# prakharg24/yoloret

Hardware: AMD Instinct MI355X
Metric: images/sec (+ p50 per-image ms) MobileNetV2-0.75x @416, 1/2/4/8 MI355X (higher is better)
Workload: dtype f32; 1 GPU; mobilenetv2x75 @416, batch 64 per GPU, fp32, random weights (SURVEY 8(d) recipe; parity tests run the variance-preserving recipe, see DESIGN.md 5), C=20: forward + decode + per-class NMS + pack; 3 steps in flight (each step = one whole batch on its own HIP stream and workspace); global_batch=64, parallelism=dp1 (image-sharded)

## Files before the change

### yoloret_amd/compiler.py

```python
import ctypes
import os

import numpy as np

from . import runtime as rt


def round_up(v, m):
    return (v + m - 1) // m * m


NO_ARENA_REUSE = os.environ.get('YOLORET_NO_ARENA_REUSE', '0') != '0'


class Buf:
    def __init__(self, bid, h, w, c, ld, external_slot=-1, name='', dtype=0):
        self.id, self.h, self.w, self.c, self.ld = bid, h, w, c, ld
        self.external_slot = external_slot
        self.name = name
        self.dtype = dtype
        self.elems = h * w * ld
        self.bytes = self.elems * rt.ESIZE[dtype]
        self.first_def = None
        self.last_use = -1
# ... 858 lines not shown
                out.append(m16)
                i += 2
            else:
                out.append(c)
                i += 1
            continue
        ok = (d is not None and c.kind == rt.OP_POINTWISE and c.dtype == 0 and c.act in ('relu6', 'none', 'swish', 'leaky') and 'scale' in c.params
              and c.res is None and not getattr(c, 'stride', 0) and not (c.se_reduced & rt.PWF_F32_MFMA) and not getattr(c, 'accounted_in', None)
              and all(s_.xform in ('identity', 'up2', 'maxpool2', 'maxpool4', 'up2_add') for s_ in c.srcs)
              and (c.gate is None or (len(c.srcs) == 1 and c.srcs[0].xform == 'identity'))
              and kp >= 16 and c.cout % 4 == 0 and c.out.external_slot < 0 and c.out.id not in output_buf_ids and readers.get(id(c.out), 0) == 1
              and d.kind == rt.OP_DEPTHWISE and d.dtype == 0 and d.k == 3 and d.stride == 1 and len(d.srcs) == 1 and d.srcs[0].buf is c.out
              and d.srcs[0].xform == 'identity' and d.srcs[0].c == c.cout and d.act in ('swish', 'relu6', 'none') and d.out.ld % 4 == 0
              and d.out.dtype == 0 and not (c.h == 1 and c.w == 1) and (d.gate is not None or FUSE_HEAD_ALL)
              and block_name(c.name) + '_head' not in nosplit)
        if not ok:
            if c.kind == rt.OP_POINTWISE and block_name(c.name) + '_head' in nosplit:
                c.se_reduced |= rt.PWF_F32_MFMA
            out.append(c)
            i += 1
            continue
        F, ldf = c.cout, round_up(c.cout, 4)
        m = OpRec(rt.OP_HEAD, block_name(c.name) + '_head', act=d.act, h=d.h, w=d.w, cin=c.cin, cout=F, k=3 | rt.ACT[c.act] << rt.HEAD_ACT_SHIFT, stride=1,
                  srcs=list(c.srcs), out=d.out, res=c.gate, macs=c.macs + d.macs, dtype=0)
        m.fused = [c, d]
        if getattr(c, 'folded_projection', None):
            m.folded_projection = c.folded_projection
        m.params = {'wgt': c.params['wgt'], 'scale': c.params['scale'], 'shift': c.params['shift']}
        dp = d.params
        kseg = [s_.c for s_ in c.srcs if s_.xform != 'up2_add']
        nk = sum((c_ + 31) // 32 for c_ in kseg)
        nt = 2 if nk <= 4 else 1
        bname_h = block_name(c.name)
        ksrc = [s_ for s_ in c.srcs if s_.xform != 'up2_add']
        hs_shape = HEAD_STREAM_ONLY or (20 <= d.h <= 30 and d.w <= 28 and nk >= 5) or (d.h < 20 and d.w <= 14 and 5 <= nk <= 8)
        stream = (HEAD_STREAM and stream_ok and hs_shape and not SE_TAIL and (not HEAD_STREAM_ONLY or bname_h in HEAD_STREAM_ONLY)
                  and all(s_.xform in ('identity', 'maxpool2', 'up2_add') for s_ in c.srcs)
                  and all(s_.xform != 'up2_add' for s_ in c.srcs[:-1]) and 1 <= len(ksrc) <= 3 and F % 32 == 0 and c.act in ('relu6', 'none')
                  and nk <= (7 if head_stream_geometry(d.h, d.w)[0] == 2 else 11) and not (c.gate is not None and (len(ksrc) != 1 or ksrc[0].xform != 'identity'))
                  and all(s_.buf.ld % 4 == 0 for s_ in ksrc)
                  and 4 * nk * 2048 + 2 * 10 * (2 if d.h >= 20 else 1) * 2048 + F * 11 * 4 + F * 4 <= 160 * 1024)
        walk = (not stream and HEAD_WALK and all(s_.xform in ('identity', 'up2_add') for s_ in c.srcs) and len(kseg) <= 3 and nk <= HEAD_WALK_MAX_NK and F % 16 == 0 and (F // 16 // nt) % 4 == 0
                and F // 16 % nt == 0 and c.act in ('relu6', 'none') and not (c.gate is not None and len(kseg) != len(c.srcs)) and F * 11 * 4 <= 64 * 1024)
        if walk or stream:
            m.k |= rt.HEAD_STREAM if stream else rt.HEAD_WALK
            cp = c.params

            def planes(wd, cp=cp, kseg=kseg, F=F):
                return head_pack((cp['wgt'][1](wd)[:F] * cp['scale'][1](wd)[:F, None]).astype(np.float32), kseg)

            def tab(wd, cp=cp, dp=dp, F=F):
                T = F // 16
                o = np.zeros((T, 11, 16), np.float32)
                o[:, :9] = (dp['wgt'][1](wd).reshape(9, -1)[:, :F] * dp['scale'][1](wd)[None, :F]).astype(np.float32).reshape(9, T, 16).transpose(1, 0, 2)
                o[:, 9], o[:, 10] = dp['shift'][1](wd)[:F].reshape(T, 16), cp['shift'][1](wd)[:F].reshape(T, 16)
                return o
            m.params = {'wgt': (((F // 16) * nk * 512,), planes), 'scale': c.params['scale'], 'wgt2': ((F // 16, 11, 16), tab)}
        elif all(s_.xform in ('identity', 'up2', 'up2_add') for s_ in c.srcs) and len(kseg) <= 3 and HEAD_DMA:
            m.k |= rt.HEAD_PLANES
            m.params['wgt'] = ((((F + 15) // 16) * nk * 512,), lambda wd, wf=c.params['wgt'][1], kseg=kseg: head_pack(wf(wd), kseg))

        def dw_rows(wd, dp=dp, F=F, ldf=ldf):
            o = np.zeros((10, ldf), np.float32)
            o[:9, :F] = (dp['wgt'][1](wd).reshape(9, -1)[:, :F] * dp['scale'][1](wd)[None, :F]).astype(np.float32)
            o[9, :F] = dp['shift'][1](wd)[:F]
            return o
        if not (walk or stream):
            m.params['wgt2'] = ((10, ldf), dw_rows)
        if d.gate is not None:
            nsy, nsx = (head_stream_rows(d.h, d.w), 1) if stream else (head_walk_rows(d.h, d.w), 1) if walk else head_regions(d.h, d.w)
            part = d.gate
            part.h, part.w = nsy * nsx, 1
            part.elems = part.h * part.w * part.ld
            part.bytes = part.elems * rt.ESIZE[part.dtype]
            m.gate, m.se_reduced = part, nsy * nsx
        if hasattr(c, 'accounting_srcs'):
            m.fused[0].accounting_srcs = c.accounting_srcs
        out.append(m)
        i += 2
    return out


def se_tail_into_producers(ops):
    producer_of_sums = {id(op.gate): op for op in ops
                        if op.gate is not None and (op.kind == rt.OP_HEAD or (op.kind == rt.OP_DEPTHWISE and not dw_uses_lds_form(op)))}
    drop = set()
    for fc in ops:
        if fc.kind != rt.OP_SE_FC or len(fc.srcs) != 1 or not fc.k > 0:
            continue
        P = producer_of_sums.get(id(fc.srcs[0].buf))
        if P is None or P.gate_out is not None or fc.out.external_slot >= 0:
            continue
        if P.kind == rt.OP_HEAD and (P.k & rt.HEAD_STREAM) == rt.HEAD_STREAM:
            continue
        C, R = fc.cin, fc.se_reduced
        ldc = round_up(C, 4)
        if C != P.cout or fc.k != P.h * P.w or ldc + R > SE_TAIL_LDS:
            continue
        fp = fc.params

        def se_w(wd, fp=fp, R=R, ldc=ldc):
            return np.concatenate([np.asarray(fp['wgt'][1](wd), np.float32).ravel(), np.asarray(fp['wgt2'][1](wd), np.float32).ravel(),
                                   np.asarray(fp['b1'][1](wd), np.float32).ravel(), np.asarray(fp['b2'][1](wd), np.float32).ravel()])
        P.params['se_w'] = ((ldc * round_up(R, 4) + R * ldc + round_up(R, 4) + ldc,), se_w)
        P.gate_out, P.se_hidden = fc.out, R
        P.macs += fc.macs
        P.absorbed = list(getattr(P, 'absorbed', ())) + [fc]
        drop.add(id(fc))
    return [op for op in ops if id(op) not in drop]



def mbr_pack(we_t, e_scale, e_shift, dw, d_scale, d_shift, wp_t, p_scale, p_shift):
    cexp = dw.shape[1] // 16 * 16
    if wp_t is None:
        wp_t, p_scale, p_shift = np.zeros((0, cexp), np.float32), np.zeros(0, np.float32), np.zeros(0, np.float32)
    cout = wp_t.shape[0]
    cin = we_t.shape[1] // 8 * 8
    assert dw.shape[1] >= cexp and cexp % 16 == 0 and cin % 16 in (0, 8), (dw.shape, we_t.shape)
    T, TO, KE, nmain = cexp // 16, (cout + 15) // 16, cin // 4, cin // 16
    wef = (we_t[:cexp, :cin] * e_scale[:cexp, None]).astype(np.float32)
    wpf = np.zeros((16 * TO, cexp), np.float32)
    wpf[:cout] = (wp_t[:, :cexp] * p_scale[:cout, None]).astype(np.float32)
    lane = np.arange(64)
    m, g = lane % 16, lane // 16
    wa = np.zeros((T, KE + 4 * TO, 64), np.float32)
    for j in range(T):
        for q in range(KE):
            c, s = divmod(q, 4)
            kidx = 16 * c + 4 * g + s if c < nmain else 16 * nmain + 2 * g + s
            wa[j, q] = wef[16 * j + m, kidx]
        for t in range(TO):
            for s in range(4):
                wa[j, KE + 4 * t + s] = wpf[16 * t + m, 16 * j + 4 * g + s]
    tab = np.zeros((T, 11, 16), np.float32)
    tab[:, :9] = (dw[:, :cexp] * d_scale[None, :cexp]).astype(np.float32).reshape(9, T, 16).transpose(1, 0, 2)
    tab[:, 9], tab[:, 10] = d_shift[:cexp].reshape(T, 16), e_shift[:cexp].reshape(T, 16)
    b2 = np.zeros(16 * TO, np.float32)
    b2[:cout] = p_shift[:cout]
    return wa, tab, b2


def mbs_wave_pairs(T, nw):
    ntl, r = divmod(T, nw)
    pairs, t0 = [], 0
    for w in range(nw):
        nt = ntl + (1 if w < r else 0)
        for q in range(0, nt, 2):
            pairs.append((t0 + q, t0 + q + 1 if q + 1 < nt else None))
        t0 += nt
    return pairs


def mbs_pack(we_t, e_scale, e_shift, dw, d_scale, d_shift, wp_t, p_scale, p_shift, nw):
    _, tab, b2 = mbr_pack(we_t, e_scale, e_shift, dw, d_scale, d_shift, wp_t, p_scale, p_shift)
    cexp = dw.shape[1] // 16 * 16
    if wp_t is None:
        wp_t, p_scale, nw = np.zeros((0, cexp), np.float32), np.zeros(0, np.float32), 0
    cout, cin = wp_t.shape[0], we_t.shape[1] // 8 * 8
    T, TO, NKE = cexp // 16, (cout + 15) // 16, (cin + 31) // 32
    wef = np.zeros((cexp, 32 * NKE), np.float32)
    wef[:, :cin] = (we_t[:cexp, :cin] * e_scale[:cexp, None]).astype(np.float32)
    wpf = np.zeros((16 * TO, cexp), np.float32)
    wpf[:cout] = (wp_t[:, :cexp] * p_scale[:cout, None]).astype(np.float32)
    assert max(np.abs(wef).max(), np.abs(wpf).max() if wpf.size else 0.0) < 60000.0, 'mbs_pack: a weight beyond the float16 range'

    def planes(x):
        h = x.astype(np.float16)
        m = ((x - h.astype(np.float32)) * np.float32(2048.0)).astype(np.float16)
        return h, m
    lane = np.arange(64)
    m_, g = lane % 16, lane // 16
    i8 = np.arange(8)
    ex = np.zeros((T, NKE, 2, 64, 8), np.float16)
    for j in range(T):
        for c in range(NKE):
            v = wef[(16 * j + m_)[:, None], 32 * c + 8 * g[:, None] + i8[None, :]]
            ex[j, c, 0], ex[j, c, 1] = planes(v)
    pairs = mbs_wave_pairs(T, nw) if nw else []
    pr = np.zeros((len(pairs), TO, 2, 64, 8), np.float16)
    for q, (ta, tb) in enumerate(pairs):
        for t in range(TO):
            v = np.zeros((64, 8), np.float32)
            v[:, :4] = wpf[(16 * t + m_)[:, None], 16 * ta + 4 * g[:, None] + i8[None, :4]]
            if tb is not None:
                v[:, 4:] = wpf[(16 * t + m_)[:, None], 16 * tb + 4 * g[:, None] + i8[None, :4]]
            pr[q, t, 0], pr[q, t, 1] = planes(v)
    wa = np.concatenate([ex.ravel(), pr.ravel()]).view(np.float32)
    return wa, tab, b2


def mbk_chunk_words(cin, cout):
    return (4 * ((cin + 31) // 32) + 2 * ((cout + 15) // 16)) * 256 + 512


def mbk_pack(we_t, e_scale, e_shift, dw, d_scale, d_shift, wp_t, p_scale, p_shift):
    wa, tab, b2 = mbs_pack(we_t, e_scale, e_shift, dw, d_scale, d_shift, wp_t, p_scale, p_shift, 1)
    cexp = dw.shape[1] // 16 * 16
    cout, cin = wp_t.shape[0], we_t.shape[1] // 8 * 8
    T, TO, NKE = cexp // 16, (cout + 15) // 16, (cin + 31) // 32
    NQ = (T + 1) // 2
    ex = wa[:T * NKE * 512].reshape(T, NKE * 512)
    pr = wa[T * NKE * 512:].reshape(NQ, TO * 512)
    cw = mbk_chunk_words(cin, cout)
    out = np.zeros((NQ, cw), np.float32)
    for q in range(NQ):
        o = 0
        for t in (2 * q, 2 * q + 1):
            if t < T:
                out[q, o:o + NKE * 512] = ex[t]
            o += NKE * 512
        out[q, o:o + TO * 512] = pr[q]
        o += TO * 512
        for t in (2 * q, 2 * q + 1):
            if t < T:
                out[q, o:o + 176] = tab[t].ravel()
            o += 176
    return out.ravel(), b2


def mbk_segs(stride, h, pad_t, nw, rows):
    ho = (h + stride - 1) // stride
    if stride == 1:
        nr = nw * rows
        return 1 if h <= nr else (h - nr + nr - 3) // (nr - 2) + 1
    s = 0
    while True:
        ylast = s * (nw - 1) + nw - 1
        end = ylast if 2 * ylast - pad_t + 2 >= h else ylast - 1
        if end >= ho - 1:
            return s + 1
        s += 1


def pad_to(fn, n, ld):
    def f(wd):
        o = np.zeros(ld, np.float32)
        o[:n] = fn(wd)[:n]
        return o
    return f


def bn_pair(prm, n, ld):
    return lambda wd: np.concatenate([pad_to(prm['scale'][1], n, ld)(wd), pad_to(prm['shift'][1], n, ld)(wd)])


def block_arrays(wd, ep, dp, pp=None):
    proj = (pp['wgt'][1](wd), pp['scale'][1](wd), pp['shift'][1](wd)) if pp is not None else (None, None, None)
    return (ep['wgt'][1](wd), ep['scale'][1](wd), ep['shift'][1](wd), dp['wgt'][1](wd).reshape(9, -1), dp['scale'][1](wd), dp['shift'][1](wd)) + proj


def packed(pack, which, ep, dp, pp=None, *extra):
    return lambda wd: pack(*block_arrays(wd, ep, dp, pp), *extra)[which]


def stem_pair_rows(prm, taps, c1p):
    def f(wd):
        sc = pad_to(prm['scale'][1], c1p, c1p)(wd)
        w = (prm['wgt'][1](wd).reshape(taps, -1)[:, :c1p] * sc[None]).astype(np.float32)
        rows = np.concatenate([w, np.ones((1, c1p), np.float32), pad_to(prm['shift'][1], c1p, c1p)(wd)[None]])
        return np.ascontiguousarray(rows.reshape(taps + 2, c1p // 2, 2).transpose(1, 0, 2)).reshape(c1p // 2, -1)
    return ((c1p // 2, (taps + 2) * 2), f)


def stemblock_params(e, d, p):
    c1p, cout, cop = round_up(e.cout, 4), p.cout, round_up(p.cout, 8)

    def proj_w(wd, pw=p.params['wgt'][1]):
        o = np.zeros((c1p, cop), np.float32)
        o[:, :cout] = pw(wd)[:, :c1p].T
        return o
    return {'wgt': stem_pair_rows(e.params, 27, c1p), 'wgt2': stem_pair_rows(d.params, 9, c1p), 'b1': ((c1p, cop), proj_w),
            'b2': ((2 * cop,), bn_pair(p.params, cout, cop))}


def stemblock_mfma_params(e, d, p, dtype):
    c1, cout = e.cout, p.cout
    c1m, com = round_up(c1, 32), round_up(cout, 16)
    korder = [g * 9 + i_ for g in range(3) for i_ in range(8)] + [i_ * 9 + 8 for i_ in range(3)]

    def stem_w(wd, ew=e.params['wgt'][1]):
        o = np.zeros((c1m, 32), np.float32)
        o[:c1, :27] = ew(wd)[korder, :c1].T
        return o

    def dw_rows(wd, dp=d.params):
        o = np.zeros((10, c1m), np.float32)
        sc = dp['scale'][1](wd)[:c1]
        o[:9, :c1] = (dp['wgt'][1](wd).reshape(9, -1)[:, :c1] * sc[None]).astype(np.float32)
        o[9, :c1] = dp['shift'][1](wd)[:c1]
        return o

    def proj_m(wd, pw=p.params['wgt'][1]):
        o = np.zeros((com, c1m), np.float32)
        o[:cout, :c1] = pw(wd)[:cout, :c1]
        return o
    return {'wgt': ((c1m, 32), stem_w, dtype), 'scale': ((c1m,), pad_to(e.params['scale'][1], c1, c1m)),
            'shift': ((c1m,), pad_to(e.params['shift'][1], c1, c1m)), 'wgt2': ((10, c1m), dw_rows), 'b1': ((com, c1m), proj_m, dtype),
            'b2': ((2 * com,), bn_pair(p.params, cout, com))}


def mbh_params(ep, dp, pp, cin, cexp, cout, k, dtype):
    kk, cexp_p, kp, ldo = k * k, round_up(cexp, 32), round_up(cin, 32), round_up(cout, 8)

    def expand_wt(wd):
        o = np.zeros((cexp_p, kp), np.float32)
        o[:cexp, :cin] = ep['wgt'][1](wd)[:, :cin]
        return o

    def chunk_params(wd):
        o = np.zeros((kk + 4, cexp_p), np.float32)
        o[:kk, :cexp] = dp['wgt'][1](wd)[:, :cexp]
        o[kk, :cexp], o[kk + 1, :cexp] = dp['scale'][1](wd)[:cexp], dp['shift'][1](wd)[:cexp]
        o[kk + 2, :cexp], o[kk + 3, :cexp] = ep['scale'][1](wd)[:cexp], ep['shift'][1](wd)[:cexp]
        return o

    def project_wt(wd):
        o = np.zeros((cout, cexp_p), np.float32)
        o[:, :cexp] = pp['wgt'][1](wd)[:, :cexp]
        return o

    def project_bn(wd):
        o = np.zeros((2, ldo), np.float32)
        o[0, :cout], o[1, :cout] = pp['scale'][1](wd)[:cout], pp['shift'][1](wd)[:cout]
        return o.ravel()
    params = {'wgt': ((cexp_p, kp), expand_wt, dtype), 'wgt2': ((kk + 4, cexp_p), chunk_params)}
    if pp is not None:
        params.update({'b1': ((cout, cexp_p), project_wt, dtype), 'b2': ((2 * ldo,), project_bn)})
    return params


def mblane_params(exp, dw, proj):
    cin, cexp, cout = (exp if exp is not None else dw).srcs[0].c, dw.cin, proj.cout
    cinp, cop, npair = round_up(cin, 4), round_up(cout, 8), round_up((cexp + 1) // 2, 8)
    e2 = 2 * npair
    ep, dwp, pp = (exp.params if exp is not None else None), dw.params, proj.params

    def pairs(rows, scale, shift):
        full = np.zeros((rows.shape[0] + 2, e2), np.float32)
        full[:-2, :cexp] = (rows[:, :cexp] * scale[None, :cexp]).astype(np.float32)
        full[-2, :cexp], full[-1, :cexp] = 1.0, shift[:cexp]
        return np.ascontiguousarray(full.reshape(-1, e2 // 2, 2).transpose(1, 0, 2)).reshape(e2 // 2, -1)

    def expand_w(wd):
        wt = ep['wgt'][1](wd)
        rows = np.zeros((cinp, wt.shape[0]), np.float32)
        rows[:wt.shape[1]] = wt.T[:cinp]
        return pairs(rows, ep['scale'][1](wd), ep['shift'][1](wd))

    def proj_w(wd):
# ... 714 lines not shown
```

### yoloret_amd/csrc/mbk.hip

```cpp
#include "yr_common.h"
#include <type_traits>

#include "mbr_common.h"

struct MbkArgs {
    const float* x; float* out;
    const float* wa;
    const float* bp;
    int H, W, Ho, Wo, ld_in, ld_out, pad_t, pad_l, strips, segs;
    unsigned wa_bytes;
};

typedef __attribute__((address_space(3))) void* mbk_lds_ptr;
#ifdef MBK_TIMING
#define MBK_T(i) { __builtin_amdgcn_sched_barrier(0); const unsigned long long t_ = __builtin_amdgcn_s_memtime(); tacc[i] += t_ - tlast; tlast = t_; __builtin_amdgcn_sched_barrier(0); }
#else
#define MBK_T(i)
#endif

template <int CIN, int CEXP, int COUT, int S, int ROWS, int NW, bool RES, int EXP = 0>
__global__ __launch_bounds__(64 * NW) void mbk_kernel(MbkArgs a) {
    constexpr int T = CEXP / 16, NQ = (T + 1) / 2, TO = (COUT + 15) / 16, NKE = (CIN + 31) / 32, NOUT = 14 / S;
    constexpr int EXB = 2 * NKE * 2 * 1024, PRB = TO * 2 * 1024, CHB = EXB + PRB + 2048;
    constexpr int NPIECE = CHB / 1024, NR = NW * ROWS;
    constexpr bool ILV = EXP != 7;
    constexpr bool SKEW = false;
    static_assert(S == 1 || ROWS == 2, "stride 2: a wave owns the two input rows of its output row");
    static_assert(CEXP % 16 == 0 && COUT % 4 == 0 && CIN % 8 == 0, "widths");
    typedef unsigned u4 __attribute__((ext_vector_type(4)));
    extern __shared__ __attribute__((aligned(16))) char lds_raw[];
    constexpr int NPR = S == 1 && ROWS > 1 ? 2 : 1;
    constexpr int XCB = (NW + 2) * NPR * 2 * 1024;
    char* const xch = lds_raw + 3 * CHB;
    const int lane = threadIdx.x & 63, px = lane & 15, mg = lane >> 4;
    const int w = __builtin_amdgcn_readfirstlane(threadIdx.x >> 6);
    int bid = (int)yr_xcd_swizzle(blockIdx.x, gridDim.x);
    const int seg = bid % a.segs; bid /= a.segs;
    const int strip = bid % a.strips;
    const int b = bid / a.strips;
#ifdef MBK_TIMING
    unsigned long long tacc[8] = {0, 0, 0, 0, 0, 0, 0, 0}, tlast = __builtin_amdgcn_s_memtime();
#endif

    int rin[ROWS];
    int yo;
    bool emit[ROWS];
    if constexpr (S == 1) {
        const int ri0 = seg * (NR - 2), out0 = seg == 0 ? 0 : ri0 + 1;
#pragma unroll
        for (int i = 0; i < ROWS; ++i) {
            const int r = ri0 + ROWS * w + i;
            rin[i] = r;
            emit[i] = r >= out0 && r < a.H && (r + 1 < ri0 + NR || r + 1 >= a.H);
        }
        yo = 0;
    } else {
        yo = seg * (NW - 1) + w;
        rin[0] = 2 * yo - a.pad_t; rin[1] = rin[0] + 1;
        emit[0] = yo < a.Ho && (w < NW - 1 || rin[0] + 2 >= a.H);
        emit[1] = false;
    }
    const int podd = S == 2 ? px >> 3 : 0;
    const int xin = S * NOUT * strip - a.pad_l + (S == 2 ? 2 * (px & 7) + podd : px);
    const int xc = min(max(xin, 0), a.W - 1);
    const bool col_in = xin >= 0 && xin < a.W;
    const int xo = NOUT * strip + (S == 2 ? (px & 7) : px - 1);
    const bool out_lane = (S == 2 ? px < 7 : (px >= 1 && px <= 14)) && xo < a.Wo;

    const yr_rsrc xsrc = yr_make_rsrc(a.x + (size_t)b * a.H * a.W * a.ld_in, (unsigned)(a.H * a.W * a.ld_in) * 4u);
    const yr_rsrc osrc = yr_make_rsrc(a.out + (size_t)b * a.Ho * a.Wo * a.ld_out, (unsigned)(a.Ho * a.Wo * a.ld_out) * 4u);
    const yr_rsrc wsrc = yr_make_rsrc(a.wa, a.wa_bytes);

    auto issue_chunk = [&](const int q) {
        char* dst = lds_raw + (q % 3) * CHB;
        const int qs = min(q, NQ - 1);
#pragma unroll
        for (int u = 0; u < (NPIECE + NW - 1) / NW; ++u) {
            const int p = u * NW + w;
            if (NPIECE % NW == 0 || p < NPIECE)
                __builtin_amdgcn_raw_ptr_buffer_load_lds(wsrc, (mbk_lds_ptr)(dst + p * 1024), 16, (unsigned)(qs * CHB + p * 1024 + lane * 16), 0, 0, 0);
        }
    };
    constexpr int NU = (NPIECE + NW - 1) / NW;
    auto issue_piece = [&](const int q, const int u) {
        const int p = u * NW + w;
        if (NPIECE % NW == 0 || p < NPIECE)
            __builtin_amdgcn_raw_ptr_buffer_load_lds(wsrc, (mbk_lds_ptr)(lds_raw + (q % 3) * CHB + p * 1024), 16, (unsigned)(min(q, NQ - 1) * CHB + p * 1024 + lane * 16), 0, 0, 0);
    };
    issue_chunk(0);
    issue_chunk(NQ > 1 ? 1 : 0);
    if (w < 2) {
#pragma unroll
        for (int u = 0; u < 2 * NPR * 2; ++u)
            reinterpret_cast<v4f*>(xch + (u / (NPR * 2)) * XCB + (w * (NW + 1) * NPR * 2 + u % (NPR * 2)) * 1024)[lane] = (v4f){0.f, 0.f, 0.f, 0.f};
    }

    v4u xh[ROWS][NKE], xm[ROWS][NKE];
    float hr[ROWS];
#pragma unroll
    for (int i = 0; i < ROWS; ++i) {
        const bool row_in = rin[i] >= 0 && rin[i] < a.H;
        hr[i] = row_in && col_in ? 6.f : 0.f;
        const unsigned so = (unsigned)min(max(rin[i], 0), a.H - 1) * (unsigned)(a.W * a.ld_in) * 4u;
        v4f lo[NKE], hi[NKE];
#pragma unroll
        for (int c = 0; c < NKE; ++c) {
            const unsigned off = 32 * c + 8 * mg < CIN ? ((unsigned)xc * (unsigned)a.ld_in + 32u * c + 8u * mg) * 4u : YR_DEAD;
            lo[c] = __builtin_bit_cast(v4f, __builtin_amdgcn_raw_buffer_load_b128(xsrc, off, so, 0));
            hi[c] = __builtin_bit_cast(v4f, __builtin_amdgcn_raw_buffer_load_b128(xsrc, off == YR_DEAD ? YR_DEAD : off + 16u, so, 0));
        }
#pragma unroll
        for (int c = 0; c < NKE; ++c) {
            const float v[8] = {lo[c][0], lo[c][1], lo[c][2], lo[c][3], hi[c][0], hi[c][1], hi[c][2], hi[c][3]};
            mbs_split8(v, xh[i][c], xm[i][c]);
        }
    }

    constexpr int NE = S == 1 ? ROWS : 1;
    v4f P[NE][TO], P1[NE][TO];
#pragma unroll
    for (int i = 0; i < NE; ++i)
#pragma unroll
        for (int t = 0; t < TO; ++t) { P[i][t] = (v4f){0.f, 0.f, 0.f, 0.f}; P1[i][t] = P[i][t]; }
    const v4f k11 = (v4f){0.00048828125f, 0.00048828125f, 0.00048828125f, 0.00048828125f};

    auto expand = [&](const char* cb, v4f (&ec)[ROWS][2]) {
        const u4* fe = reinterpret_cast<const u4*>(cb) + lane;
        const v4f* tb0 = reinterpret_cast<const v4f*>(cb + EXB + PRB) + mg;
#pragma unroll
        for (int j = 0; j < 2; ++j) {
            const v4f se = tb0[44 * j + 40];
            v4f e1[ROWS];
#pragma unroll
            for (int i = 0; i < ROWS; ++i) { ec[i][j] = se; e1[i] = (v4f){0.f, 0.f, 0.f, 0.f}; }
#pragma unroll
            for (int c = 0; c < NKE; ++c) {
                if (EXP == 2) continue;
                const u4 wh = EXP == 6 ? xh[0][c] : fe[((j * NKE + c) * 2 + 0) * 64], wm = EXP == 6 ? xm[0][c] : fe[((j * NKE + c) * 2 + 1) * 64];
#pragma unroll
                for (int i = 0; i < ROWS; ++i) ec[i][j] = mbs_mfma(wh, xh[i][c], ec[i][j]);
#pragma unroll
                for (int i = 0; i < ROWS; ++i) e1[i] = mbs_mfma(wh, xm[i][c], e1[i]);
#pragma unroll
                for (int i = 0; i < ROWS; ++i) e1[i] = mbs_mfma(wm, xh[i][c], e1[i]);
            }
#pragma unroll
            for (int i = 0; i < ROWS; ++i) {
                ec[i][j] = __builtin_elementwise_fma(e1[i], k11, ec[i][j]);
#pragma unroll
                for (int s = 0; s < 4; ++s) ec[i][j][s] = __builtin_amdgcn_fmed3f(ec[i][j][s], 0.f, hr[i]);
            }
        }
    };
    auto park_rows = [&](const int q, const v4f (&ec)[ROWS][2]) {
        v4f* park = reinterpret_cast<v4f*>(xch + (q & 1) * XCB) + lane;
#pragma unroll
        for (int j = 0; j < 2; ++j) {
            park[(((w + 1) * NPR + 0) * 2 + j) * 64] = ec[0][j];
            if (NPR > 1) park[(((w + 1) * NPR + 1) * 2 + j) * 64] = ec[ROWS - 1][j];
        }
    };
    auto dw_project = [&](const int q, const char* cb, const v4f (&ec)[ROWS][2]) {
        const u4* fp = reinterpret_cast<const u4*>(cb + EXB) + lane;
        const v4f* tb0 = reinterpret_cast<const v4f*>(cb + EXB + PRB) + mg;
        const v4f* park = reinterpret_cast<const v4f*>(xch + (q & 1) * XCB) + lane;
        v4f above[2], below[2];
#pragma unroll
        for (int j = 0; j < 2; ++j) {
            above[j] = S == 1 ? park[((w * NPR + NPR - 1) * 2 + j) * 64] : (v4f){0.f, 0.f, 0.f, 0.f};
            below[j] = park[(((w + 2) * NPR + 0) * 2 + j) * 64];
        }
        v4f d[NE][2];
#pragma unroll
        for (int j = 0; j < 2; ++j) {
            const v4f* tb = tb0 + 44 * j;
            if constexpr (S == 1) {
#pragma unroll
                for (int i = 0; i < ROWS; ++i) d[i][j] = tb[36];
#pragma unroll
                for (int ky = 0; ky < 3; ++ky) {
                    const v4f w0 = tb[12 * ky], w1 = tb[12 * ky + 4], w2 = tb[12 * ky + 8];
#pragma unroll
                    for (int i = 0; i < ROWS; ++i) {
                        const int rr = i + ky - 1;
                        if (EXP == 1) { d[i][j] += (rr < 0 ? above[j] : rr >= ROWS ? below[j] : ec[rr < 0 ? 0 : rr >= ROWS ? 0 : rr][j]) * w1; continue; }
                        mbr_dw_row(d[i][j], rr < 0 ? above[j] : rr >= ROWS ? below[j] : ec[rr < 0 ? 0 : rr >= ROWS ? 0 : rr][j], w0, w1, w2);
                    }
                }
            } else {
                d[0][j] = tb[36];
                mbr_dw_row2<false>(d[0][j], ec[0][j], tb[0], tb[4], tb[8]);
                mbr_dw_row2<false>(d[0][j], ec[1][j], tb[12], tb[16], tb[20]);
                mbr_dw_row2<false>(d[0][j], below[j], tb[24], tb[28], tb[32]);
            }
#pragma unroll
            for (int i = 0; i < NE; ++i)
#pragma unroll
                for (int s = 0; s < 4; ++s) d[i][j][s] = yr_relu6_fast(d[i][j][s]);
        }
        v4u bh[NE], bm[NE];
#pragma unroll
        for (int i = 0; i < NE; ++i) {
            const float v[8] = {d[i][0][0], d[i][0][1], d[i][0][2], d[i][0][3], d[i][1][0], d[i][1][1], d[i][1][2], d[i][1][3]};
            mbs_split8(v, bh[i], bm[i]);
        }
#pragma unroll
        for (int t = 0; t < TO; ++t) {
            if (EXP == 3) { P[0][t] += __builtin_bit_cast(v4f, bh[0]) + __builtin_bit_cast(v4f, bm[NE - 1]); continue; }
            const u4 wh = EXP == 6 ? bm[0] : fp[(t * 2 + 0) * 64], wm = EXP == 6 ? bh[0] : fp[(t * 2 + 1) * 64];
#pragma unroll
            for (int i = 0; i < NE; ++i) P[i][t] = mbs_mfma(wh, bh[i], P[i][t]);
#pragma unroll
            for (int i = 0; i < NE; ++i) P1[i][t] = mbs_mfma(wh, bm[i], P1[i][t]);
#pragma unroll
            for (int i = 0; i < NE; ++i) P1[i][t] = mbs_mfma(wm, bh[i], P1[i][t]);
        }
    };

    auto fused_step = [&](const int q, const char* cbq, const char* cbn, const v4f (&ec)[ROWS][2], v4f (&en)[ROWS][2]) {
        constexpr int MPG = 3 * ROWS, NMG = 2 * NKE, NM = NMG * MPG;
        constexpr int PPG = 3 * NE, NDG = 6, NV = NDG * PPG;
        constexpr int NS = NM > NV ? NM : NV;
        const u4* fe = reinterpret_cast<const u4*>(cbn) + lane;
        const v4f* tbn = reinterpret_cast<const v4f*>(cbn + EXB + PRB) + mg;
        const u4* fp = reinterpret_cast<const u4*>(cbq + EXB) + lane;
        const v4f* tbq = reinterpret_cast<const v4f*>(cbq + EXB + PRB) + mg;
        const v4f* park = reinterpret_cast<const v4f*>(xch + (q & 1) * XCB) + lane;
        v4f above[2], below[2], d[NE][2], e1[ROWS];
        u4 fr[2][2];
        v4f tp[2][3];
#pragma unroll
        for (int j = 0; j < 2; ++j) {
            above[j] = S == 1 ? park[((w * NPR + NPR - 1) * 2 + j) * 64] : (v4f){0.f, 0.f, 0.f, 0.f};
            below[j] = park[(((w + 2) * NPR + 0) * 2 + j) * 64];
        }
        fr[0][0] = fe[0]; fr[0][1] = fe[64];
        tp[0][0] = tbq[0]; tp[0][1] = tbq[4]; tp[0][2] = tbq[8];
#pragma unroll
        for (int j = 0; j < 2; ++j) {
            const v4f sh = tbq[44 * j + 36], se = tbn[44 * j + 40];
#pragma unroll
            for (int i = 0; i < NE; ++i) d[i][j] = sh;
#pragma unroll
            for (int i = 0; i < ROWS; ++i) en[i][j] = se;
        }
        __builtin_amdgcn_sched_barrier(0);
        MBK_T(2)
        mbk_for<NS>([&](auto SS) {
            constexpr int sl = decltype(SS)::value;
            if constexpr (EXP != 5) {
                mbk_for<NU>([&](auto UU) {
                    constexpr int u = decltype(UU)::value;
                    if constexpr ((2 * u + 1) * NS / (2 * NU) == sl) issue_piece(q + 2, u);
                });
            }
            if constexpr (sl < NM) {
                constexpr int g = sl / MPG, r = sl % MPG, kind = r / ROWS, i = r % ROWS, j = g / NKE, c = g % NKE;
                if constexpr (r == 0 && g + 1 < NMG) {
                    fr[(g + 1) & 1][0] = fe[((g + 1) * 2 + 0) * 64];
                    fr[(g + 1) & 1][1] = fe[((g + 1) * 2 + 1) * 64];
                }
                if constexpr (c == 0 && kind == 1) e1[i] = (v4f){0.f, 0.f, 0.f, 0.f};
                if constexpr (EXP == 2) {}
                else if constexpr (kind == 0) en[i][j] = mbs_mfma(fr[g & 1][0], xh[i][c], en[i][j]);
                else if constexpr (kind == 1) e1[i] = mbs_mfma(fr[g & 1][0], xm[i][c], e1[i]);
                else e1[i] = mbs_mfma(fr[g & 1][1], xh[i][c], e1[i]);
                if constexpr (c == NKE - 1 && kind == 2) en[i][j] = __builtin_elementwise_fma(e1[i], k11, en[i][j]);
            }
            if constexpr (sl < NV) {
                constexpr int dg = sl / PPG, pr = sl % PPG, i = pr / 3, part = pr % 3, j = dg / 3, ky = dg % 3;
                if constexpr (pr == 0 && dg + 1 < NDG) {
                    constexpr int j1 = (dg + 1) / 3, ky1 = (dg + 1) % 3;
                    tp[(dg + 1) & 1][0] = tbq[44 * j1 + 12 * ky1];
                    tp[(dg + 1) & 1][1] = tbq[44 * j1 + 12 * ky1 + 4];
                    tp[(dg + 1) & 1][2] = tbq[44 * j1 + 12 * ky1 + 8];
                }
                if constexpr (EXP == 1) { if (part == 0) d[i][j] += ec[i][j] * tp[dg & 1][1] + above[j] + below[j]; }
                else if constexpr (S == 1) {
                    constexpr int rr = i + ky - 1;
                    mbk_dw_part(part, d[i][j], rr < 0 ? above[j] : rr >= ROWS ? below[j] : ec[rr < 0 ? 0 : rr >= ROWS ? 0 : rr][j], tp[dg & 1][part == 0 ? 1 : part == 1 ? 0 : 2]);
                } else {
                    mbk_dw2_part(part, d[0][j], ky == 0 ? ec[0][j] : ky == 1 ? ec[1][j] : below[j], tp[dg & 1][part]);
                }
            }
            __builtin_amdgcn_sched_barrier(0);
        });
        MBK_T(3)
        u4 pf[2][2];
        pf[0][0] = fp[0]; pf[0][1] = fp[64];
        v4u bh[NE], bm[NE];
#pragma unroll
        for (int i = 0; i < NE; ++i) {
#pragma unroll
            for (int j = 0; j < 2; ++j)
#pragma unroll
                for (int s = 0; s < 4; ++s) d[i][j][s] = yr_relu6_fast(d[i][j][s]);
            const float v[8] = {d[i][0][0], d[i][0][1], d[i][0][2], d[i][0][3], d[i][1][0], d[i][1][1], d[i][1][2], d[i][1][3]};
            mbs_split8(v, bh[i], bm[i]);
        }
        __builtin_amdgcn_sched_barrier(0);
        MBK_T(4)
        constexpr int MPT = 3 * NE, NM3 = TO * MPT, NV3 = ROWS * 2;
        mbk_for<(NM3 > NV3 ? NM3 : NV3)>([&](auto SS) {
            constexpr int sl = decltype(SS)::value;
            if constexpr (sl < NM3) {
                constexpr int t = sl / MPT, r = sl % MPT, kind = r / NE, i = r % NE;
                if constexpr (r == 0 && t + 1 < TO) {
                    pf[(t + 1) & 1][0] = fp[((t + 1) * 2 + 0) * 64];
                    pf[(t + 1) & 1][1] = fp[((t + 1) * 2 + 1) * 64];
                }
                if constexpr (EXP == 3) { if (kind == 0) P[i][t] += __builtin_bit_cast(v4f, bh[i] + pf[t & 1][0]) + __builtin_bit_cast(v4f, bm[i] + pf[t & 1][1]); }
                else if constexpr (kind == 0) P[i][t] = mbs_mfma(pf[t & 1][0], bh[i], P[i][t]);
                else if constexpr (kind == 1) P1[i][t] = mbs_mfma(pf[t & 1][0], bm[i], P1[i][t]);
                else P1[i][t] = mbs_mfma(pf[t & 1][1], bh[i], P1[i][t]);
            }
            if constexpr (sl < NV3) {
                constexpr int i = sl / 2, j = sl % 2;
#pragma unroll
                for (int s = 0; s < 4; ++s) en[i][j][s] = __builtin_amdgcn_fmed3f(en[i][j][s], 0.f, hr[i]);
            }
            __builtin_amdgcn_sched_barrier(0);
        });
        MBK_T(5)
    };

    v4f ec[ROWS][2];
    __builtin_amdgcn_s_waitcnt(yr_waitcnt_imm(0, YR_LGKM_ANY));
    __syncthreads();
    expand(lds_raw, ec);
    park_rows(0, ec);
    MBK_T(0)
    for (int q = 0; q + 1 < NQ; ++q) {
        __builtin_amdgcn_s_waitcnt(yr_waitcnt_imm(0, YR_LGKM_ANY));
        if (EXP != 4) __syncthreads();
        MBK_T(1)
        if (EXP != 5 && !ILV) issue_chunk(q + 2);
        v4f en[ROWS][2];
        if (ILV) {
            fused_step(q, lds_raw + (q % 3) * CHB, lds_raw + ((q + 1) % 3) * CHB, ec, en);
        } else if (SKEW && (w & 4)) {
            expand(lds_raw + ((q + 1) % 3) * CHB, en);
            __builtin_amdgcn_sched_barrier(0);
            dw_project(q, lds_raw + (q % 3) * CHB, ec);
        } else {
            dw_project(q, lds_raw + (q % 3) * CHB, ec);
            __builtin_amdgcn_sched_barrier(0);
            expand(lds_raw + ((q + 1) % 3) * CHB, en);
        }
        park_rows(q + 1, en);
#pragma unroll
        for (int i = 0; i < ROWS; ++i) { ec[i][0] = en[i][0]; ec[i][1] = en[i][1]; }
        MBK_T(6)
    }
    v4f res[NE][RES ? TO : 1], psh[TO];
    unsigned oaddr[NE];
#pragma unroll
    for (int i = 0; i < NE; ++i) {
        const int y = S == 1 ? rin[i] : yo;
        const bool live = emit[i] && out_lane;
        const unsigned opix = ((unsigned)max(y, 0) * (unsigned)a.Wo + (unsigned)xo);
        oaddr[i] = live ? opix * (unsigned)a.ld_out * 4u : YR_DEAD;
        if constexpr (RES) {
#pragma unroll
            for (int t = 0; t < TO; ++t)
                res[i][t] = __builtin_bit_cast(v4f, __builtin_amdgcn_raw_buffer_load_b128(xsrc, live && 16 * t + 4 * mg < COUT ? (opix * (unsigned)a.ld_in + 16u * t + 4u * mg) * 4u : YR_DEAD, 0, 0));
        }
    }
#pragma unroll
    for (int t = 0; t < TO; ++t) psh[t] = *reinterpret_cast<const v4f*>(a.bp + 16 * t + 4 * mg);
    __builtin_amdgcn_sched_barrier(0);
    __syncthreads();
    dw_project(NQ - 1, lds_raw + ((NQ - 1) % 3) * CHB, ec);

#pragma unroll
    for (int i = 0; i < NE; ++i) {
#pragma unroll
        for (int t = 0; t < TO; ++t) {
            const int co = 16 * t + 4 * mg;
            v4f v = __builtin_elementwise_fma(P1[i][t], k11, P[i][t]) + psh[t];
            if constexpr (RES) v += res[i][t];
            __builtin_amdgcn_raw_buffer_store_b128(__builtin_bit_cast(u4, v), osrc, oaddr[i] != YR_DEAD && co < COUT ? oaddr[i] + (unsigned)co * 4u : YR_DEAD, 0, 0);
        }
    }
#ifdef MBK_TIMING
    MBK_T(7)
    __builtin_amdgcn_s_waitcnt(yr_waitcnt_imm(0, YR_LGKM_ANY));
    if (lane < 8) reinterpret_cast<unsigned*>(a.out)[(size_t)(gridDim.x / (a.strips * a.segs)) * a.Ho * a.Wo * a.ld_out + ((size_t)blockIdx.x * NW + w) * 8 + lane] = (unsigned)tacc[lane];
#endif
}

static int mbk_segs(int S, int H, int Ho, int pad_t, int NW, int ROWS) {
    if (S == 1) {
        const int NR = NW * ROWS;
        return H <= NR ? 1 : (H - NR + NR - 3) / (NR - 2) + 1;
    }
    int s = 0;
    for (;; ++s) {
        const int ylast = s * (NW - 1) + NW - 1;
        const int end = (2 * ylast - pad_t + 2 >= H) ? ylast : ylast - 1;
        if (end >= Ho - 1) break;
    }
    return s + 1;
}

template <int CIN, int CEXP, int COUT, int S, int ROWS, int NW, bool RES, int EXP = 0>
static int launch_mbk(const MbkArgs& a0, int batch, hipStream_t s) {
    MbkArgs a = a0;
    constexpr int T = CEXP / 16, NQ = (T + 1) / 2, TO = (COUT + 15) / 16, NKE = (CIN + 31) / 32, NOUT = 14 / S;
    constexpr int CHB = 2 * NKE * 2 * 1024 + TO * 2 * 1024 + 2048;
    a.strips = (a.Wo + NOUT - 1) / NOUT;
    a.segs = mbk_segs(S, a.H, a.Ho, a.pad_t, NW, ROWS);
    a.wa_bytes = (unsigned)NQ * CHB;
    const size_t lds = (size_t)3 * CHB + (size_t)2 * (NW + 2) * (S == 1 && ROWS > 1 ? 2 : 1) * 2 * 1024;
    return ch_launch<mbk_kernel<CIN, CEXP, COUT, S, ROWS, NW, RES, EXP>>(dim3((unsigned)(batch * a.strips * a.segs)), dim3(64 * NW), lds, lds, s, a,
                                                                         "mbk_kernel<%d,%d,%d,%d,%d,%d,%d>", CIN, CEXP, COUT, S, ROWS, NW, (int)RES);
}

int yr_launch_mbk(const yr_op& op, int batch, hipStream_t s) {
    YR_REQUIRE(op.dtype == YR_F32 && op.out_dtype == YR_F32, "mbk: float32 plans only");
    YR_REQUIRE(op.nsrc == 1 && op.src[0].xform == YR_X_IDENTITY && op.src[0].dtype == YR_F32, "mbk: needs one float32 identity source");
// ... 42 lines not shown
```

### yoloret_amd/csrc/mbr_common.h

```cpp
#pragma once
#include "chained_common.h"
#include <type_traits>

#define MBR_TAB 176

__device__ __forceinline__ float mbr_shr1(float v) {
    return __int_as_float(__builtin_amdgcn_update_dpp(0, __float_as_int(v), 0x111, 0xf, 0xf, true));
}
__device__ __forceinline__ float mbr_shl1(float v) {
    return __int_as_float(__builtin_amdgcn_update_dpp(0, __float_as_int(v), 0x101, 0xf, 0xf, true));
}

__device__ __forceinline__ void mbr_dw_row(v4f& acc, const v4f e, const v4f w0, const v4f w1, const v4f w2) {
    acc = __builtin_elementwise_fma(e, w1, acc);
    float a0 = acc[0], a1 = acc[1], a2 = acc[2], a3 = acc[3];
    asm("s_nop 1\n\t" CH_FMAC_DPP(w0, CH_DPP("row_shr:1")) CH_FMAC_DPP(w2, CH_DPP("row_shl:1"))
        : CH_ACC4(a, a) : CH_IN4(e, e), CH_IN4(w0, w0), CH_IN4(w2, w2));
    acc = (v4f){a0, a1, a2, a3};
}

template <bool ODD>
__device__ __forceinline__ void mbr_dw_row2(v4f& acc, const v4f e, const v4f w0, const v4f w1, const v4f w2) {
    float a0 = acc[0], a1 = acc[1], a2 = acc[2], a3 = acc[3];
    if constexpr (!ODD) CH_PAIR3(CH_OWN, "row_shl:8", "row_shl:1", "0x3", w0, w1, w2);
    else CH_PAIR3("row_shr:8", CH_OWN, "row_shr:7", "0xc", w0, w1, w2);
    acc = (v4f){a0, a1, a2, a3};
}

typedef _Float16 mbs_h2 __attribute__((ext_vector_type(2)));
typedef _Float16 mbs_h8 __attribute__((ext_vector_type(8)));
__device__ __forceinline__ void mbs_split8(const float (&v)[8], v4u& h, v4u& m) {
#pragma unroll
    for (int p = 0; p < 4; ++p) {
        unsigned hh, mm;
        yr_cut2(v[2 * p], v[2 * p + 1], hh, mm);
        h[p] = hh;
        m[p] = mm;
    }
}
__device__ __forceinline__ v4f mbs_mfma(v4u a, v4u b, v4f c) {
    return __builtin_amdgcn_mfma_f32_16x16x32_f16(__builtin_bit_cast(mbs_h8, a), __builtin_bit_cast(mbs_h8, b), c, 0, 0, 0);
}

template <int N, class F>
__device__ __forceinline__ void mbk_for(F&& f) {
    if constexpr (N > 0) {
        mbk_for<N - 1>(f);
        f(std::integral_constant<int, N - 1>{});
    }
}

#define MBK_TAP(mods) asm(CH_FMAC_DPP(wt, mods) : CH_ACC4(a, a) : CH_IN4(e, e), CH_IN4(wt, wt))
__device__ __forceinline__ void mbk_dw_part(const int part, v4f& acc, const v4f e, const v4f wt) {
    if (part == 0) { acc = __builtin_elementwise_fma(e, wt, acc); return; }
    float a0 = acc[0], a1 = acc[1], a2 = acc[2], a3 = acc[3];
    if (part == 1) MBK_TAP(CH_DPP("row_shr:1"));
    else MBK_TAP(CH_DPP("row_shl:1"));
    acc = (v4f){a0, a1, a2, a3};
}
__device__ __forceinline__ void mbk_dw2_part(const int part, v4f& acc, const v4f e, const v4f wt) {
    float a0 = acc[0], a1 = acc[1], a2 = acc[2], a3 = acc[3];
    if (part == 0) MBK_TAP(CH_DPPM(CH_OWN, "0x3"));
    else if (part == 1) MBK_TAP(CH_DPPM("row_shl:8", "0x3"));
    else MBK_TAP(CH_DPPM("row_shl:1", "0x3"));
    acc = (v4f){a0, a1, a2, a3};
}
#undef MBK_TAP

static inline int hw_seg_rows(int H) { return H <= 16 ? H : (H + ((H + 12) / 13) - 1) / ((H + 12) / 13); }
```

Measured before the change: 51980 img/s.

## Pack split-fp16 correction terms into idle K lanes of last expansion MFMA chunk

When the input channel count leaves the last 32-wide K chunk only one or two groups of 8 filled, the packer copies the weight hi-plane into the unused lane groups of the mid-plane. The kernel then loads input channels so that the idle groups carry the low-part correction, scaled through v_fma_mix. That lets a single MFMA compute both cross terms of the split-precision product for that chunk, dropping one of three MFMAs per row on the tail chunk. It adds per-lane select logic and a new split routine, and depends on host and device agreeing on the lane layout.

```diff
diff --git a/yoloret_amd/compiler.py b/yoloret_amd/compiler.py
--- a/yoloret_amd/compiler.py
+++ b/yoloret_amd/compiler.py
@@ -1034,7 +1034,12 @@
     return pairs
 
 
-def mbs_pack(we_t, e_scale, e_shift, dw, d_scale, d_shift, wp_t, p_scale, p_shift, nw):
+def mbs_cross_tail(cin):
+    tg = cin // 8 % 4
+    return tg if tg in (1, 2) else 0
+
+
+def mbs_pack(we_t, e_scale, e_shift, dw, d_scale, d_shift, wp_t, p_scale, p_shift, nw, dense=False):
     _, tab, b2 = mbr_pack(we_t, e_scale, e_shift, dw, d_scale, d_shift, wp_t, p_scale, p_shift)
     cexp = dw.shape[1] // 16 * 16
     if wp_t is None:
@@ -1059,6 +1064,10 @@
         for c in range(NKE):
             v = wef[(16 * j + m_)[:, None], 32 * c + 8 * g[:, None] + i8[None, :]]
             ex[j, c, 0], ex[j, c, 1] = planes(v)
+    tg = mbs_cross_tail(cin) if dense else 0
+    if tg:
+        lanes = ex.reshape(T, NKE, 2, 4, 16, 8)
+        lanes[:, NKE - 1, 1, tg:2 * tg] = lanes[:, NKE - 1, 0, :tg]
     pairs = mbs_wave_pairs(T, nw) if nw else []
     pr = np.zeros((len(pairs), TO, 2, 64, 8), np.float16)
     for q, (ta, tb) in enumerate(pairs):
@@ -1077,7 +1086,7 @@
 
 
 def mbk_pack(we_t, e_scale, e_shift, dw, d_scale, d_shift, wp_t, p_scale, p_shift):
-    wa, tab, b2 = mbs_pack(we_t, e_scale, e_shift, dw, d_scale, d_shift, wp_t, p_scale, p_shift, 1)
+    wa, tab, b2 = mbs_pack(we_t, e_scale, e_shift, dw, d_scale, d_shift, wp_t, p_scale, p_shift, 1, dense=True)
     cexp = dw.shape[1] // 16 * 16
     cout, cin = wp_t.shape[0], we_t.shape[1] // 8 * 8
     T, TO, NKE = cexp // 16, (cout + 15) // 16, (cin + 31) // 32
diff --git a/yoloret_amd/csrc/mbk.hip b/yoloret_amd/csrc/mbk.hip
--- a/yoloret_amd/csrc/mbk.hip
+++ b/yoloret_amd/csrc/mbk.hip
@@ -23,6 +23,7 @@
     constexpr int T = CEXP / 16, NQ = (T + 1) / 2, TO = (COUT + 15) / 16, NKE = (CIN + 31) / 32, NOUT = 14 / S;
     constexpr int EXB = 2 * NKE * 2 * 1024, PRB = TO * 2 * 1024, CHB = EXB + PRB + 2048;
     constexpr int NPIECE = CHB / 1024, NR = NW * ROWS;
+    constexpr int TG = mbs_cross_tail(CIN), NX = TG ? 2 * NKE - 1 : 2 * NKE;
     constexpr bool ILV = EXP != 7;
     constexpr bool SKEW = false;
     static_assert(S == 1 || ROWS == 2, "stride 2: a wave owns the two input rows of its output row");
@@ -95,6 +96,8 @@
             reinterpret_cast<v4f*>(xch + (u / (NPR * 2)) * XCB + (w * (NW + 1) * NPR * 2 + u % (NPR * 2)) * 1024)[lane] = (v4f){0.f, 0.f, 0.f, 0.f};
     }
 
+    const int xg = mbs_cross_group(TG, mg);
+    const float xcm = mg < TG ? 1.f : -2048.f, xsm = mg < TG ? 0.f : 2048.f;
     v4u xh[ROWS][NKE], xm[ROWS][NKE];
     float hr[ROWS];
 #pragma unroll
@@ -105,14 +108,21 @@
         v4f lo[NKE], hi[NKE];
 #pragma unroll
         for (int c = 0; c < NKE; ++c) {
-            const unsigned off = 32 * c + 8 * mg < CIN ? ((unsigned)xc * (unsigned)a.ld_in + 32u * c + 8u * mg) * 4u : YR_DEAD;
+            const int cg = TG && c == NKE - 1 ? xg : (32 * c + 8 * mg < CIN ? mg : -1);
+            const unsigned off = cg >= 0 ? ((unsigned)xc * (unsigned)a.ld_in + 32u * c + 8u * cg) * 4u : YR_DEAD;
             lo[c] = __builtin_bit_cast(v4f, __builtin_amdgcn_raw_buffer_load_b128(xsrc, off, so, 0));
             hi[c] = __builtin_bit_cast(v4f, __builtin_amdgcn_raw_buffer_load_b128(xsrc, off == YR_DEAD ? YR_DEAD : off + 16u, so, 0));
         }
 #pragma unroll
         for (int c = 0; c < NKE; ++c) {
             const float v[8] = {lo[c][0], lo[c][1], lo[c][2], lo[c][3], hi[c][0], hi[c][1], hi[c][2], hi[c][3]};
-            mbs_split8(v, xh[i][c], xm[i][c]);
+            if (TG && c == NKE - 1) {
+                mbs_split8_cross(v, xcm, xsm, xh[i][c], xm[i][c]);
+#pragma unroll
+                for (int p = 0; p < 4; ++p) xh[i][c][p] = mg < TG ? xh[i][c][p] : 0u;
+            } else {
+                mbs_split8(v, xh[i][c], xm[i][c]);
+            }
         }
     }
 
@@ -139,6 +149,11 @@
                 const u4 wh = EXP == 6 ? xh[0][c] : fe[((j * NKE + c) * 2 + 0) * 64], wm = EXP == 6 ? xm[0][c] : fe[((j * NKE + c) * 2 + 1) * 64];
 #pragma unroll
                 for (int i = 0; i < ROWS; ++i) ec[i][j] = mbs_mfma(wh, xh[i][c], ec[i][j]);
+                if (TG && c == NKE - 1) {
+#pragma unroll
+                    for (int i = 0; i < ROWS; ++i) e1[i] = mbs_mfma(wm, xm[i][c], e1[i]);
+                    continue;
+                }
 #pragma unroll
                 for (int i = 0; i < ROWS; ++i) e1[i] = mbs_mfma(wh, xm[i][c], e1[i]);
 #pragma unroll
@@ -218,7 +233,7 @@
     };
 
     auto fused_step = [&](const int q, const char* cbq, const char* cbn, const v4f (&ec)[ROWS][2], v4f (&en)[ROWS][2]) {
-        constexpr int MPG = 3 * ROWS, NMG = 2 * NKE, NM = NMG * MPG;
+        constexpr int MPG = 3 * ROWS, NMG = 2 * NKE, MPT_E = (NKE + NX) * ROWS, NM = 2 * MPT_E;
         constexpr int PPG = 3 * NE, NDG = 6, NV = NDG * PPG;
         constexpr int NS = NM > NV ? NM : NV;
         const u4* fe = reinterpret_cast<const u4*>(cbn) + lane;
@@ -255,7 +270,8 @@
                 });
             }
             if constexpr (sl < NM) {
-                constexpr int g = sl / MPG, r = sl % MPG, kind = r / ROWS, i = r % ROWS, j = g / NKE, c = g % NKE;
+                constexpr int j = sl / MPT_E, rt = sl % MPT_E, c = rt / MPG < NKE - 1 ? rt / MPG : NKE - 1, r = rt - c * MPG, g = j * NKE + c, kind = r / ROWS, i = r % ROWS;
+                constexpr bool dense = TG && c == NKE - 1;
                 if constexpr (r == 0 && g + 1 < NMG) {
                     fr[(g + 1) & 1][0] = fe[((g + 1) * 2 + 0) * 64];
                     fr[(g + 1) & 1][1] = fe[((g + 1) * 2 + 1) * 64];
@@ -263,9 +279,9 @@
                 if constexpr (c == 0 && kind == 1) e1[i] = (v4f){0.f, 0.f, 0.f, 0.f};
                 if constexpr (EXP == 2) {}
                 else if constexpr (kind == 0) en[i][j] = mbs_mfma(fr[g & 1][0], xh[i][c], en[i][j]);
-                else if constexpr (kind == 1) e1[i] = mbs_mfma(fr[g & 1][0], xm[i][c], e1[i]);
+                else if constexpr (kind == 1) e1[i] = mbs_mfma(fr[g & 1][dense ? 1 : 0], xm[i][c], e1[i]);
                 else e1[i] = mbs_mfma(fr[g & 1][1], xh[i][c], e1[i]);
-                if constexpr (c == NKE - 1 && kind == 2) en[i][j] = __builtin_elementwise_fma(e1[i], k11, en[i][j]);
+                if constexpr (c == NKE - 1 && kind == (dense ? 1 : 2)) en[i][j] = __builtin_elementwise_fma(e1[i], k11, en[i][j]);
             }
             if constexpr (sl < NV) {
                 constexpr int dg = sl / PPG, pr = sl % PPG, i = pr / 3, part = pr % 3, j = dg / 3, ky = dg % 3;
diff --git a/yoloret_amd/csrc/mbr_common.h b/yoloret_amd/csrc/mbr_common.h
--- a/yoloret_amd/csrc/mbr_common.h
+++ b/yoloret_amd/csrc/mbr_common.h
@@ -38,6 +38,23 @@
         m[p] = mm;
     }
 }
+static constexpr __host__ __device__ int mbs_cross_tail(int cin) { return (cin / 8) % 4 == 1 || (cin / 8) % 4 == 2 ? (cin / 8) % 4 : 0; }
+static __device__ __forceinline__ int mbs_cross_group(int tg, int mg) { return mg < tg ? mg : mg < 2 * tg ? mg - tg : -1; }
+__device__ __forceinline__ void mbs_split8_cross(const float (&v)[8], const float cm, const float sm, v4u& h, v4u& x) {
+    typedef float cut_f2 __attribute__((ext_vector_type(2)));
+    typedef _Float16 cut_h2 __attribute__((ext_vector_type(2)));
+#pragma unroll
+    for (int p = 0; p < 4; ++p) {
+        const cut_f2 xv = (cut_f2){v[2 * p], v[2 * p + 1]};
+        const unsigned hh = __builtin_bit_cast(unsigned, __builtin_convertvector(xv, cut_h2));
+        const cut_f2 xs = xv * sm;
+        unsigned mm;
+        asm("v_fma_mixlo_f16 %0, %1, %2, %3 op_sel_hi:[1,0,0]" : "=v"(mm) : "v"(hh), "v"(cm), "v"(xs[0]));
+        asm("v_fma_mixhi_f16 %0, %1, %2, %3 op_sel:[1,0,0] op_sel_hi:[1,0,0]\n\ts_nop 1" : "+v"(mm) : "v"(hh), "v"(cm), "v"(xs[1]));
+        h[p] = hh;
+        x[p] = mm;
+    }
+}
 __device__ __forceinline__ v4f mbs_mfma(v4u a, v4u b, v4f c) {
     return __builtin_amdgcn_mfma_f32_16x16x32_f16(__builtin_bit_cast(mbs_h8, a), __builtin_bit_cast(mbs_h8, b), c, 0, 0, 0);
 }
```

Result: no change. 51570 img/s (-0.8%).
